# hkust-vgd/scanobjectnn

Measured on AMD Instinct MI355X. Metric: point-clouds/sec fwd+bwd at B×2048×3, 15-cls, higher is better.
Workload: dtype f32

## Files before the change

include/pcops.h:

```cpp
#ifndef PCOPS_H
#define PCOPS_H

#ifdef __cplusplus
extern "C" {
#endif

typedef void *pcops_stream_t;

typedef struct pcops_rows {
    const void *blocks;
    const int *block_start;
    const int *rows;
} pcops_rows_t;

typedef enum pcops_status {
    PCOPS_OK = 0,
    PCOPS_ERR_NULL_POINTER = -1,
    PCOPS_ERR_BAD_SHAPE = -2,
    PCOPS_ERR_BAD_ARGUMENT = -3,
    PCOPS_ERR_UNSUPPORTED = -4,
    PCOPS_ERR_LAUNCH = -5
} pcops_status;

const char *pcops_strerror(int status);
int pcops_abi_version(void);

typedef enum pcops_option {
    PCOPS_OPT_GEMM_SPLIT_BF16 = 1,
    PCOPS_OPT_WGRAD_SPLIT_BF16 = 2,
    PCOPS_OPT_BWD_FUSED_DX_SPLIT_BF16 = 3,
    PCOPS_OPT_KNN_F16_PREFILTER = 4,
    PCOPS_OPT_DGRAD_SPLIT_BF16 = 5,
    PCOPS_OPT_BWD_FUSED_GRAM_WGRAD = 6,
    PCOPS_OPT_SCATTER_QFORM = 7,
    PCOPS_OPT_XYZ_STATS_MOMENTS = 8,
    PCOPS_OPT_GRAM_SPLIT_BF16 = 9,
    PCOPS_OPT_POOL_TOP_ROWS_PIPELINED = 10,
    PCOPS_OPT_XCONV_CHANNEL_GROUPS = 11,
    PCOPS_OPT_COUNT = 12
} pcops_option;
int pcops_set_option(int option, int value);
int pcops_get_option(int option);
int pcops_last_launch_pipe(void);
int pcops_last_launch_plan(int *out, int n);
int pcops_last_launch_acc_stats(void);

int pcops_farthest_point_sample(int b, int n, int m, const float *inp, float *temp,
                                int *out, pcops_stream_t stream);
unsigned long long pcops_farthest_point_sample_workspace_bytes(int b, int n);

int pcops_prob_sample(int b, int n, int m, const float *inp_p, const float *inp_r, float *temp,
                      int *out, pcops_stream_t stream);

int pcops_gather_point(int b, int n, int m, const float *inp, const int *idx,
                       float *out, pcops_stream_t stream);
int pcops_gather_point_grad(int b, int n, int m, const float *out_g, const int *idx,
                            float *inp_g, pcops_stream_t stream);

int pcops_query_ball_point(int b, int n, int m, float radius, int nsample,
                           const float *xyz1, const float *xyz2, int *idx,
                           int *pts_cnt, pcops_stream_t stream);

int pcops_query_ball_point_multi(int b, int n, int m, int nscale, const float *radius,
                                 const int *nsample, const float *xyz1,
                                 const float *xyz2, int *const *idx,
                                 int *const *pts_cnt, pcops_stream_t stream);

int pcops_group_point(int b, int n, int c, int m, int nsample, const float *points,
                      const int *idx, float *out, pcops_stream_t stream);
int pcops_group_point_grad(int b, int n, int c, int m, int nsample,
                           const float *grad_out, const int *idx, float *grad_points,
                           pcops_stream_t stream);

int pcops_selection_sort(int b, int n, int m, int k, const float *dist, int *outi,
                         float *out, pcops_stream_t stream);
int pcops_knn_point_supported(int n);
int pcops_knn_point(int b, int n, int c, int m, int k, const float *xyz1, const float *xyz2, float *val, int *idx,
                    pcops_stream_t stream);
int pcops_knn_point_dist(int b, int n, int c, int m, const float *xyz1, const float *xyz2, float *dist,
                         pcops_stream_t stream);

int pcops_three_nn(int b, int n, int m, const float *xyz1, const float *xyz2,
                   float *dist, int *idx, pcops_stream_t stream);
int pcops_three_interpolate(int b, int m, int c, int n, const float *points,
                            const int *idx, const float *weight, float *out,
                            pcops_stream_t stream);
int pcops_three_interpolate_grad(int b, int n, int c, int m, const float *grad_out,
                                 const int *idx, const float *weight,
                                 float *grad_points, pcops_stream_t stream);

void pcops_set_deterministic(int on);
int pcops_get_deterministic(void);
// ... 415 lines not shown
```

scanobjectnn_amd/_lib.py:

```python
import ctypes as C
import os
import re
import weakref

import torch

_HERE = os.path.dirname(os.path.abspath(__file__))
LIB_PATH = os.environ.get("PCOPS_LIB") or os.path.join(_HERE, "libpcops.so")

_I, _F, _P, _U64, _LL = C.c_int, C.c_float, C.c_void_p, C.c_ulonglong, C.c_longlong
ABI_VERSION = 4

HEADER_PATH = os.path.join(os.path.dirname(_HERE), "include", "pcops.h")


class PcopsError(RuntimeError):
    pass


_SCALARS = {"int": _I, "float": _F, "long long": _LL, "unsigned long long": _U64}


def _ctype(decl, fn):
    if "*" in decl:
# ... 101 lines not shown
def load():
    global _lib
    if _lib is not None:
        return _lib
    if not os.path.exists(LIB_PATH):
        raise PcopsError(
            "libpcops.so is missing (%s). Build it with `python -c 'import __graft_entry__ as g; "
            "g.build()'` or `make -C scanobjectnn_amd/csrc`. There is no CPU fallback." % LIB_PATH)
    lib = C.CDLL(LIB_PATH)
    for name, (argtypes, _) in SIGNATURES.items():
        fn = getattr(lib, name)
        fn.argtypes = list(argtypes) + [_P]
        fn.restype = _I
    for name, (argtypes, restype) in PLAIN.items():
        fn = getattr(lib, name)
        fn.argtypes = argtypes
        fn.restype = restype
    got = int(lib.pcops_abi_version())
    if got != ABI_VERSION:
        raise PcopsError("%s reports ABI version %d, this binding is written for %d: rebuild it "
                         "(make -C scanobjectnn_amd/csrc)" % (LIB_PATH, got, ABI_VERSION))
    _lib = lib
    return lib


def strerror(status):
    return load().pcops_strerror(int(status)).decode()


def ptr(t):
    return t.data_ptr() if t is not None else None


def check(t, dtype, name, ndim=None):
    if not isinstance(t, torch.Tensor):
        raise TypeError("%s must be a torch.Tensor" % name)
    if not t.is_cuda:
        raise PcopsError("%s is on %s: pcops ops run on the MI355X only (no CPU fallback)"
                         % (name, t.device))
    if t.dtype != dtype:
        raise TypeError("%s must be %s, got %s" % (name, dtype, t.dtype))
    if ndim is not None and t.dim() != ndim:
        raise ValueError("%s must have rank %d, got shape %s" % (name, ndim, tuple(t.shape)))
    return t.contiguous()


OPT_GEMM_SPLIT_BF16, OPT_WGRAD_SPLIT_BF16, OPT_BWD_FUSED_DX_SPLIT_BF16, OPT_KNN_F16_PREFILTER = 1, 2, 3, 4
OPT_DGRAD_SPLIT_BF16, OPT_BWD_FUSED_GRAM_WGRAD = 5, 6
OPT_SCATTER_QFORM = 7
OPT_XYZ_STATS_MOMENTS = 8
OPT_GRAM_SPLIT_BF16 = 9
OPT_POOL_TOP_ROWS_PIPELINED = 10
OPT_XCONV_CHANNEL_GROUPS = 11


def set_option(option, value):
    prev = int(load().pcops_set_option(int(option), int(value)))
    if prev < 0:
        raise PcopsError("pcops_set_option(%d, %d): %s" % (option, value, strerror(prev)))
    return prev


def get_option(option):
    return int(load().pcops_get_option(int(option)))


def set_deterministic(on=True):
    load().pcops_set_deterministic(1 if on else 0)


def deterministic():
    return bool(load().pcops_get_deterministic())


def scatter_rows_sorted_supported(rows, ndst):
    return bool(load().pcops_scatter_rows_sorted_supported(int(rows), int(ndst)))


def scatter_rows_sorted(idx, src, ndst, div=1, w=None, out=None, c=None, ld=None, src_ptr=None):
    b, rows = idx.shape[0], idx[0].numel()
    if not scatter_rows_sorted_supported(rows, ndst):
        raise PcopsError("ordered scatter-add (deterministic backward): %d destination points per cloud, the limit is "
                         "%d (the per-cloud counting sort lives in LDS); rows %d must stay below 2^30.  Switch "
                         "deterministic mode off for clouds this large." % (ndst, load().pcops_scatter_rows_sorted_max_ndst(), rows))
    if c is None:
        c, ld = src.shape[-1], src.shape[-1]
    acc = out is not None
    if out is None:
        out = torch.empty((b, ndst, c), dtype=torch.float32, device=idx.device)
    ws = torch.empty(int(load().pcops_scatter_rows_workspace_bytes(b, rows, ndst)) // 8 + 1, dtype=torch.int64,
                     device=idx.device)
    call("pcops_scatter_rows_sorted", b, rows, ndst, c, div, ld, idx.data_ptr(), ptr(w),
         src_ptr if src_ptr is not None else src.data_ptr(), out.data_ptr(), 1 if acc else 0, ws.data_ptr())
    return out


def scatter_grouped(dfg, idx, n):
    b, m, k, c = dfg.shape
    if deterministic():
        return scatter_rows_sorted(idx.view(b, m * k), dfg.view(b, m * k, c), n)
    out = torch.empty((b, n, c), dtype=torch.float32, device=dfg.device)
    call("pcops_group_point_grad", b, n, c, m, k, dfg.data_ptr(), idx.data_ptr(), out.data_ptr())
    return out


_SYNC_EVERY_CALL = os.environ.get("PCOPS_SYNC", "0") == "1"
# ... 19 lines not shown
```

scanobjectnn_amd/csrc/abi.hip:

```cpp
#include <atomic>
#include <cstdint>
#include <cstdlib>

#include "common.h"

extern "C" const char *pcops_strerror(int status) {
    switch (status) {
        case PCOPS_OK: return "ok";
        case PCOPS_ERR_NULL_POINTER: return "null pointer argument";
        case PCOPS_ERR_BAD_SHAPE: return "invalid tensor extents";
        case PCOPS_ERR_BAD_ARGUMENT: return "invalid attribute (radius/nsample/npoint/k)";
        case PCOPS_ERR_UNSUPPORTED: return "shape outside the range the gfx950 kernels are built for";
        case PCOPS_ERR_LAUNCH: return "HIP launch failed";
        default: return "unknown pcops status";
    }
}

extern "C" int pcops_abi_version(void) { return 4; }

static std::atomic<int> g_deterministic{pcops_env_switch("PCOPS_DETERMINISTIC", false) ? 1 : 0};
extern "C" void pcops_set_deterministic(int on) { g_deterministic.store(on ? 1 : 0); }

namespace {
int env_opt(const char *name, int dflt, int hi) {
    const int v = pcops_env_int(name, dflt);
    return v < 0 ? 0 : (v > hi ? hi : v);
}
std::atomic<int> g_options[PCOPS_OPT_COUNT] = {};
std::atomic<int> g_options_init{0};
void options_init() {
    if (g_options_init.load(std::memory_order_acquire)) return;
    static std::atomic_flag busy = ATOMIC_FLAG_INIT;
    while (busy.test_and_set(std::memory_order_acquire)) {}
    if (!g_options_init.load(std::memory_order_relaxed)) {
        g_options[PCOPS_OPT_GEMM_SPLIT_BF16].store(env_opt("PCOPS_GEMM_BF3", 1, 2));
        g_options[PCOPS_OPT_WGRAD_SPLIT_BF16].store(pcops_env_int("PCOPS_WGRAD_BF3", 1) != 0);
        g_options[PCOPS_OPT_BWD_FUSED_DX_SPLIT_BF16].store(env_opt("PCOPS_BWD_FUSED_DX3", 2, 2));
        g_options[PCOPS_OPT_KNN_F16_PREFILTER].store(pcops_env_int("PCOPS_KNN_F16", 1) != 0);
        g_options[PCOPS_OPT_DGRAD_SPLIT_BF16].store(env_opt("PCOPS_DGRAD_BF3", 1, 2));
        g_options[PCOPS_OPT_BWD_FUSED_GRAM_WGRAD].store(pcops_env_int("PCOPS_BWD_FUSED_GW", 0) != 0);
        g_options[PCOPS_OPT_SCATTER_QFORM].store(pcops_env_int("PCOPS_SCATTER_QFORM", 1) != 0);
        g_options[PCOPS_OPT_XYZ_STATS_MOMENTS].store(pcops_env_int("PCOPS_XYZ_STATS_MOMENTS", 0) != 0);
        g_options[PCOPS_OPT_GRAM_SPLIT_BF16].store(pcops_env_int("PCOPS_GRAM_BF3", 1) != 0);
        g_options[PCOPS_OPT_POOL_TOP_ROWS_PIPELINED].store(pcops_env_int("PCOPS_POOL_TOP_ROWS_PIPE", 1) != 0);
        g_options[PCOPS_OPT_XCONV_CHANNEL_GROUPS].store(pcops_env_int("PCOPS_XCONV_GROUPS", 1) != 0);
        g_options_init.store(1, std::memory_order_release);
    }
    busy.clear(std::memory_order_release);
}
}

extern "C" int pcops_get_option(int option) {
    if (option <= 0 || option >= PCOPS_OPT_COUNT) return PCOPS_ERR_BAD_ARGUMENT;
    options_init();
    return g_options[option].load();
}

extern "C" int pcops_set_option(int option, int value) {
    if (option <= 0 || option >= PCOPS_OPT_COUNT || value < 0) return PCOPS_ERR_BAD_ARGUMENT;
    if ((option == PCOPS_OPT_GEMM_SPLIT_BF16 || option == PCOPS_OPT_DGRAD_SPLIT_BF16 ||
         option == PCOPS_OPT_BWD_FUSED_DX_SPLIT_BF16) ? value > 2 : value > 1)
        return PCOPS_ERR_BAD_ARGUMENT;
    options_init();
    return g_options[option].exchange(value);
}
extern "C" int pcops_get_deterministic(void) { return g_deterministic.load(); }

static thread_local int t_last_pipe = 0;
static thread_local int t_last_acc_stats = 0;
void pcops_note_pipe(int pipe) { t_last_pipe = pipe; t_last_acc_stats = 0; }
void pcops_note_acc_stats(int on) { t_last_acc_stats = on; }
extern "C" int pcops_last_launch_pipe(void) { return t_last_pipe; }
extern "C" int pcops_last_launch_acc_stats(void) { return t_last_acc_stats; }

static thread_local int t_last_plan[5] = {0, 0, 0, 0, 0};
void pcops_note_plan(int path, int split, int bn, int wst, int pool) {
    t_last_plan[0] = path; t_last_plan[1] = split; t_last_plan[2] = bn; t_last_plan[3] = wst; t_last_plan[4] = pool;
    t_last_acc_stats = 0;
}
void pcops_note_plan_field(int field, int value) {
    if (field >= 0 && field < 5) t_last_plan[field] = value;
}
extern "C" int pcops_last_launch_plan(int *out, int n) {
    if (!out || n < 0) return PCOPS_ERR_NULL_POINTER;
    for (int i = 0; i < n && i < 5; ++i) out[i] = t_last_plan[i];
    return 5;
}

namespace {
__global__ __launch_bounds__(256) void adam_step_kernel(long long n4, float4 *__restrict__ p, const float4 *__restrict__ g,
                                                        float4 *__restrict__ m, float4 *__restrict__ v, float b1, float b2,
                                                        float lr_t, float eps) {
    const float c1 = 1.f - b1, c2 = 1.f - b2;
    for (long long i = (long long)blockIdx.x * 256 + threadIdx.x; i < n4; i += (long long)gridDim.x * 256) {
        const float4 gi = g[i];
        float4 mi = m[i], vi = v[i], pi = p[i];
        mi.x = fmaf(c1, gi.x, b1 * mi.x); mi.y = fmaf(c1, gi.y, b1 * mi.y);
        mi.z = fmaf(c1, gi.z, b1 * mi.z); mi.w = fmaf(c1, gi.w, b1 * mi.w);
        vi.x = fmaf(c2 * gi.x, gi.x, b2 * vi.x); vi.y = fmaf(c2 * gi.y, gi.y, b2 * vi.y);
        vi.z = fmaf(c2 * gi.z, gi.z, b2 * vi.z); vi.w = fmaf(c2 * gi.w, gi.w, b2 * vi.w);
        pi.x -= lr_t * mi.x / (sqrtf(vi.x) + eps); pi.y -= lr_t * mi.y / (sqrtf(vi.y) + eps);
        pi.z -= lr_t * mi.z / (sqrtf(vi.z) + eps); pi.w -= lr_t * mi.w / (sqrtf(vi.w) + eps);
        m[i] = mi; v[i] = vi; p[i] = pi;
    }
}
__global__ __launch_bounds__(256) void adam_step_dev_kernel(long long n4, float4 *__restrict__ p, const float4 *__restrict__ g,
                                                            float4 *__restrict__ m, float4 *__restrict__ v, float b1, float b2,
                                                            const float *__restrict__ lr_t_dev, float eps) {
    const float c1 = 1.f - b1, c2 = 1.f - b2;
    const float lr_t = *lr_t_dev;
    for (long long i = (long long)blockIdx.x * 256 + threadIdx.x; i < n4; i += (long long)gridDim.x * 256) {
        const float4 gi = g[i];
        float4 mi = m[i], vi = v[i], pi = p[i];
        mi.x = fmaf(c1, gi.x, b1 * mi.x); mi.y = fmaf(c1, gi.y, b1 * mi.y);
// ... 45 lines not shown
```

scanobjectnn_amd/csrc/common.h:

```cpp
#pragma once
#include <hip/hip_runtime.h>
#include <stdint.h>
#include <stdio.h>
#include <stdlib.h>

#include <type_traits>

#include "../../include/pcops.h"
#include "device.h"

#define PCOPS_REQUIRE_PTR(p) \
    do { if ((p) == nullptr) return PCOPS_ERR_NULL_POINTER; } while (0)
#define PCOPS_REQUIRE_SHAPE(cond) \
    do { if (!(cond)) return PCOPS_ERR_BAD_SHAPE; } while (0)
#define PCOPS_REQUIRE_ARG(cond) \
    do { if (!(cond)) return PCOPS_ERR_BAD_ARGUMENT; } while (0)

static inline bool pcops_env_switch(const char *name, bool dflt) {
    const char *e = getenv(name);
    return dflt ? !(e && e[0] == '0') : (e && e[0] == '1');
}
static inline int pcops_env_int(const char *name, int dflt) {
    const char *e = getenv(name);
    return e ? atoi(e) : dflt;
// ... 5 lines not shown
    static const bool verbose = getenv("PCOPS_DEBUG_LAUNCH") != nullptr;
    if (verbose) fprintf(stderr, "libpcops: launch failed: %s (%s)\n", hipGetErrorString(e), hipGetErrorName(e));
    return PCOPS_ERR_LAUNCH;
}

static inline hipStream_t as_stream(pcops_stream_t s) { return reinterpret_cast<hipStream_t>(s); }

static inline unsigned cdiv(long long a, long long b) { return (unsigned)((a + b - 1) / b); }

static __global__ __launch_bounds__(256) void pcops_zero_kernel(unsigned *__restrict__ p, size_t n) {
    for (size_t i = (size_t)blockIdx.x * 256 + threadIdx.x; i < n; i += (size_t)gridDim.x * 256) p[i] = 0u;
}
static inline hipError_t pcops_zero_async(void *p, size_t bytes, hipStream_t st) {
    hipStreamCaptureStatus capturing = hipStreamCaptureStatusNone;
    if (st == nullptr || bytes == 0 || (bytes & 3) || (reinterpret_cast<uintptr_t>(p) & 3) ||
        hipStreamIsCapturing(st, &capturing) != hipSuccess || capturing != hipStreamCaptureStatusActive)
        return hipMemsetAsync(p, 0, bytes, st);
    const size_t n = bytes / 4;
    const unsigned grid = n < (size_t)4096 * 256 ? cdiv((long long)n, 256) : 4096u;
    hipLaunchKernelGGL(pcops_zero_kernel, dim3(grid), dim3(256), 0, st, static_cast<unsigned *>(p), n);
    return hipGetLastError();
}

template <typename... Params, typename... Args>
static inline int pcops_launch_lds(void (*kern)(Params...), dim3 grid, dim3 block, size_t lds, int max_lds, hipStream_t st,
                                   Args... args) {
    if (hipFuncSetAttribute(reinterpret_cast<const void *>(kern), hipFuncAttributeMaxDynamicSharedMemorySize, max_lds) !=
        hipSuccess)
        return PCOPS_ERR_LAUNCH;
    hipLaunchKernelGGL(kern, grid, block, lds, st, args...);
    return pcops_launch_status();
}

template <int... Vs, typename F>
static inline int pcops_dispatch(int v, int otherwise, F &&f) {
    int rc = otherwise;
    (void)((v == Vs && ((rc = f(std::integral_constant<int, Vs>{})), true)) || ...);
    return rc;
}

extern "C" int pcops_get_deterministic(void);
extern "C" int pcops_get_option(int option);
void pcops_note_pipe(int pipe);
void pcops_note_acc_stats(int on);
void pcops_note_plan(int path, int split, int bn, int wst, int pool);
void pcops_note_plan_field(int field, int value);

bool pcops_xyz_bwd_tiles_form(long long M, int K, int N);
int pcops_xyz_bwd_tiles_launch(long long M, int groups, const float *off4, const float *xyzw, const float *a_scale,
                               const float *a_shift, const float *G, const float *Y, const float *p, const float *q,
                               const float *t, const float *W, float *partial, float *dW, float *db, float *stats_partial,
                               float *xyz_stats, hipStream_t st);

constexpr int kWave = 64;

#ifndef PCOPS_WAVE_PRIO
#define PCOPS_WAVE_PRIO 0
#endif
__device__ __forceinline__ void wave_prio_stagger() {
#if PCOPS_WAVE_PRIO & 1
    const unsigned slot = __builtin_amdgcn_s_getreg((3 << 11) | (0 << 6) | 4);
    if (slot & 1) __builtin_amdgcn_s_setprio(1);
#endif
}
__device__ __forceinline__ void wave_prio_consumer(bool consumer) {
#if PCOPS_WAVE_PRIO & 2
    if (consumer) __builtin_amdgcn_s_setprio(1);
#else
    (void)consumer;
#endif
}

__device__ __forceinline__ unsigned wave_max_u32(unsigned v) {
    auto step = [&](auto ctrl, auto rmask) {
        const unsigned o = (unsigned)__builtin_amdgcn_update_dpp(0, (int)v, decltype(ctrl)::value, decltype(rmask)::value,
                                                                 0xf, true);
        v = o > v ? o : v;
    };
    step(std::integral_constant<int, 0x111>{}, std::integral_constant<int, 0xf>{});
    step(std::integral_constant<int, 0x112>{}, std::integral_constant<int, 0xf>{});
    step(std::integral_constant<int, 0x114>{}, std::integral_constant<int, 0xf>{});
    step(std::integral_constant<int, 0x118>{}, std::integral_constant<int, 0xf>{});
    step(std::integral_constant<int, 0x142>{}, std::integral_constant<int, 0xa>{});
    step(std::integral_constant<int, 0x143>{}, std::integral_constant<int, 0xc>{});
    return (unsigned)__builtin_amdgcn_readlane((int)v, 63);
}

__device__ __forceinline__ unsigned long long wave_max_u64(unsigned long long v) {
    const unsigned hi = (unsigned)(v >> 32), lo = (unsigned)(v & 0xffffffffu);
    const unsigned mh = wave_max_u32(hi);
    const unsigned ml = wave_max_u32(hi == mh ? lo : 0u);
    return ((unsigned long long)mh << 32) | ml;
}

__device__ __forceinline__ unsigned xcd_contiguous(unsigned bid, unsigned nwg) {
    const unsigned q = nwg >> 3, r = nwg & 7u, x = bid & 7u, i = bid >> 3;
    return (x < r ? x * (q + 1) : r * (q + 1) + (x - r) * q) + i;
}
struct CloudPart { int part, cloud; };
__device__ __forceinline__ CloudPart xcd_cloud_part() {
    const unsigned vb = xcd_contiguous(blockIdx.x + blockIdx.y * gridDim.x, gridDim.x * gridDim.y);
    const unsigned cloud = vb / gridDim.x;
    return CloudPart{(int)(vb - cloud * gridDim.x), (int)cloud};
}
```

scanobjectnn_amd/csrc/mlp.hip:

```cpp
#include <stdlib.h>

#include "common.h"
#include <initializer_list>
#include <type_traits>

#ifndef PCOPS_MLP_PART
#define PCOPS_MLP_PART (-1)
#endif
#define PCOPS_PART(p_) (PCOPS_MLP_PART < 0 || PCOPS_MLP_PART == (p_))
#define PCOPS_HIDDEN __attribute__((visibility("hidden")))

#ifndef PCOPS_BF_RM
#define PCOPS_BF_RM 1
#endif

namespace pcops_mlp {

constexpr int kBM = 128;
constexpr int kBK = 32;
constexpr int kLdA = 36;

enum AMode { A_PLAIN = 0, A_BNRELU = 1, A_DY = 2, A_DYPOOL = 3, A_DYPOOLU = 4 };
constexpr int A_DYPOOLB = 6;
constexpr int A_DYW = 7;
// ... 5593 lines not shown
    GemmArgs a = fwd_args(M, K, N, nullptr, K, pro_scale, pro_shift, W, bias, Y, stats_partial, stat_pivot);
    a.off4 = off4; a.xw = xyzw; a.xw_ld = K;
    if (const int rc = set_rows(a, rows)) return rc;
    return launch_gemm_ws_only<A_XYZ, E_FWD>(a, as_stream(stream));
}

int pcops_mlp_gemm_dgrad_xyz(int M, int K, int Nout, const float *G, const float *Y, const float *p,
                             const float *q, const float *t, const float *gpool, const unsigned char *argmax,
                             int S, const float *pool_scale, const float *pool_shift, const float *Wt,
                             const float *off4, const float *xyzw, const float *prev_scale,
                             const float *prev_shift, float *Gprev, float *stats_partial, float *xyz_stats,
                             pcops_stream_t stream) {
    return pcops_mlp_gemm_dgrad_xyz_rows(M, K, Nout, G, Y, p, q, t, gpool, argmax, S, pool_scale, pool_shift, Wt, off4,
                                         xyzw, prev_scale, prev_shift, Gprev, stats_partial, xyz_stats, nullptr, stream);
}

int pcops_mlp_gemm_dgrad_xyz_rows(int M, int K, int Nout, const float *G, const float *Y, const float *p,
                                  const float *q, const float *t, const float *gpool, const unsigned char *argmax,
                                  int S, const float *pool_scale, const float *pool_shift, const float *Wt,
                                  const float *off4, const float *xyzw, const float *prev_scale,
                                  const float *prev_shift, float *Gprev, float *stats_partial, float *xyz_stats,
                                  const pcops_rows_t *rows, pcops_stream_t stream) {
    PCOPS_REQUIRE_SHAPE(M >= 1 && K >= 4 && K % 4 == 0 && Nout >= 1);
    PCOPS_REQUIRE_PTR(Y); PCOPS_REQUIRE_PTR(p); PCOPS_REQUIRE_PTR(q); PCOPS_REQUIRE_PTR(t);
    PCOPS_REQUIRE_PTR(Wt); PCOPS_REQUIRE_PTR(off4); PCOPS_REQUIRE_PTR(xyzw);
    PCOPS_REQUIRE_ARG(Gprev != nullptr || xyz_stats != nullptr);
    if (xyz_stats) PCOPS_REQUIRE_PTR(stats_partial);
    PCOPS_REQUIRE_PTR(prev_scale); PCOPS_REQUIRE_PTR(prev_shift);
    if (reinterpret_cast<uintptr_t>(off4) & 15) return PCOPS_ERR_UNSUPPORTED;
    GemmArgs a = {};
    a.M = M; a.K = K; a.N = Nout; a.X = G; a.X2 = Y; a.ldx = K; a.v0 = p; a.v1 = q; a.v2 = t;
    a.v3 = pool_scale; a.v4 = pool_shift; a.gpool = gpool; a.argmax = argmax; a.S = S > 0 ? S : 1;
    a.W = Wt; a.Y = Gprev; a.ldy = Nout; a.msc = prev_scale; a.msh = prev_shift;
    a.off4 = off4; a.xw = xyzw; a.xw_ld = Nout;
    a.stats = stats_partial; a.xstats = xyz_stats;
    if (const int rc = set_rows(a, rows)) return rc;
    hipStream_t st = as_stream(stream);
    if (gpool) {
        PCOPS_REQUIRE_PTR(argmax); PCOPS_REQUIRE_PTR(pool_scale); PCOPS_REQUIRE_PTR(pool_shift);
        a.X = Y;
        return launch_gemm_ws_only<A_DYPOOL, E_MASKX>(a, st);
    }
    PCOPS_REQUIRE_PTR(G);
    return launch_gemm_ws_only<A_DY, E_MASKX>(a, st);
}


static int gram_full_groups(long long M, int K, int ldx, const void *X) {
    if (!gram_full_on() || !ws_enabled() || M < 65536 || K > 320 || K < 32 || K % 4 != 0 || ldx % 4 != 0) return 0;
    if (reinterpret_cast<uintptr_t>(X) & 15) return 0;
    return clamp_groups(256, (M + 31) / 32);
}

int pcops_mlp_wgrad_splits(long long M, int K, int N) {
    WgradPlan pl;
    int best = wgrad_legacy_splits(M, K, N);
    for (const int g : {wgrad_pc_tile(K, N, false, &pl), wgrad_pc_tile(K, N, true, &pl), wgrad_bf3_tile(K, N, &pl),
                        wgrad_ws_tile(K, N, &pl)})
        if (g > best) best = g;
    if (K == N && gram_full_groups(M, K, 4, nullptr) > best) best = gram_full_groups(M, K, 4, nullptr);
    return best;
}

int pcops_gather_stack_rows_supported(int b, int n, int m, int s, int has_q, int nlayers, const int *widths) {
    if (b < 1 || m < 1 || s < kBlk || s % kBlk != 0 || s > 256 || nlayers < 2 || !widths) return 0;
    if (!ws_enabled() || !wgrad_pc_enabled()) return 0;
    const long long M = (long long)b * m * s;
    if (M > 0x7fffffffll) return 0;
    for (int l = 1; l < nlayers; ++l) {
        const int K = widths[l - 1], N = widths[l];
        GemmArgs f = {};
        f.M = (int)M; f.K = K; f.N = N; f.ldx = K; f.ldy = N;
        GemmArgs d = {};
        d.M = (int)M; d.K = N; d.N = K; d.ldx = N; d.ldy = K; d.S = s;
        WsPlan pl;
        if (!ws_plan(f, A_BNRELU, &pl) || !ws_plan(d, A_DY, &pl) || !wgrad_pc_shape_ok(M, K, N, K)) return 0;
    }
    if (has_q && !pcops_sa_scatter_rows_supported(n, m, s, widths[0])) return 0;
    return 1;
}

static int bwd_fused_groups(long long M, int K, int N, int S, int pooled) {
    if (!ws_enabled() || !wgrad_pc_enabled()) return 0;
    static const bool on = pcops_env_switch("PCOPS_BWD_FUSED", true);
    if (!on) return 0;
    if (M < 65536 || M > 0x7fffff00ll || K > 64 || K % 4 != 0 || N > 128 || N % 4 != 0) return 0;
    if (pooled && (S < 1 || S > 255)) return 0;
    return clamp_groups(256, (M + 31) / 32);
}

int pcops_mlp_bwd_fused_groups(long long M, int K, int N, int S, int pooled) { return bwd_fused_groups(M, K, N, S, pooled); }

int pcops_mlp_bwd_fused(long long M, int K, int N, const float *Yprev, const float *a_scale, const float *a_shift,
                        const float *G, const float *Y, const float *p, const float *q, const float *t,
                        const float *gpool, const unsigned char *argmax, int S, const float *W, float *partial,
                        float *dW, float *db, float *Gprev, float *stats_partial, pcops_stream_t stream) {
    return pcops_mlp_bwd_fused_rows(M, K, N, Yprev, a_scale, a_shift, G, Y, p, q, t, gpool, argmax, S, W, partial, dW, db,
                                    Gprev, stats_partial, nullptr, stream);
}


static int bwd_fused_gw_groups(long long M, int K, int N, int S) {
    if (pcops_get_option(PCOPS_OPT_BWD_FUSED_GRAM_WGRAD) == 0 || S < 11 || S > 255) return 0;
    if (pcops_get_option(PCOPS_OPT_BWD_FUSED_DX_SPLIT_BF16) == 0) return 0;
    return bwd_fused_groups(M, K, N, S, 1);
}
// ... 184 lines not shown
    if (!dgrad_top_plan(M, Kp, &pl)) return 0;
    if (!(wgrad_pc_enabled() && wgrad_pc_shape_ok(M, Kp, Kp, Kp, true))) return 0;
    const long long slots = (long long)(M / S) * (S < N ? S : N);
    return slots * Kp * 4 < (long long)kOOB ? 1 : 0;
}

int pcops_mlp_pool_top_addend(int M, int Kp, int N, int S, const float *gout, const float *ysel,
                            const unsigned char *argmax, const float *pool_scale, const float *pool_shift,
                            const float *p, const float *Wt, float *addend, int *rowmap, pcops_stream_t stream) {
    PCOPS_REQUIRE_SHAPE(M >= 1 && S >= 1 && S <= 256 && M % S == 0 && Kp % 4 == 0 && N >= 1 && N <= 65535);
    PCOPS_REQUIRE_PTR(gout); PCOPS_REQUIRE_PTR(ysel); PCOPS_REQUIRE_PTR(argmax); PCOPS_REQUIRE_PTR(pool_scale);
    PCOPS_REQUIRE_PTR(pool_shift); PCOPS_REQUIRE_PTR(p); PCOPS_REQUIRE_PTR(Wt); PCOPS_REQUIRE_PTR(addend);
    PCOPS_REQUIRE_PTR(rowmap);
    if (reinterpret_cast<uintptr_t>(Wt) & 15 || reinterpret_cast<uintptr_t>(addend) & 15) return PCOPS_ERR_UNSUPPORTED;
    if (N > 1024 || Kp > 512) return PCOPS_ERR_UNSUPPORTED;
    if (M / S <= 512)
        hipLaunchKernelGGL(pool_top_addend_kernel<1024>, dim3(M / S), dim3(1024), 0, as_stream(stream), S, N, Kp,
                           S < N ? S : N, gout, ysel, argmax, pool_scale, pool_shift, p, Wt, addend, rowmap);
    else
        hipLaunchKernelGGL(pool_top_addend_kernel<256>, dim3(M / S), dim3(256), 0, as_stream(stream), S, N, Kp,
                           S < N ? S : N, gout, ysel, argmax, pool_scale, pool_shift, p, Wt, addend, rowmap);
    return pcops_launch_status();
}

int pcops_mlp_gemm_dgrad_top(int M, int Kp, const float *Yprev, const float *prev_scale, const float *prev_shift,
                             const float *Mq, const float *vconst, const float *addend, long long addend_rows,
                             const int *rowmap, float *Gprev, float *stats_partial, pcops_stream_t stream) {
    return pcops_mlp_gemm_dgrad_top_rows(M, Kp, Yprev, prev_scale, prev_shift, Mq, vconst, addend, addend_rows, rowmap, Gprev,
                                         stats_partial, nullptr, stream);
}

static int gram_finish(const GramArgs &g, int gg, float *gram, float *xsum, hipStream_t st) {
    const long long L = (long long)g.K * g.K;
    hipLaunchKernelGGL(sum_partials2_kernel, dim3(cdiv(L, 64) + (xsum ? cdiv(g.K, 64) : 0)), dim3(1024), 0, st, gg, L,
                       g.part, gram, (long long)g.K, g.xpart, xsum);
    hipLaunchKernelGGL(mirror_lower_kernel, dim3(g.K), dim3(256), 0, st, g.K, gram);
    return pcops_launch_status();
}

int pcops_mlp_gram(long long M, int Kp, const float *Yprev, int ldx, const float *a_scale, const float *a_shift,
                   float *partial, float *gram, float *xsum, pcops_stream_t stream) {
    PCOPS_REQUIRE_SHAPE(M >= 1 && Kp >= 1 && ldx >= Kp);
    PCOPS_REQUIRE_PTR(Yprev); PCOPS_REQUIRE_PTR(partial); PCOPS_REQUIRE_PTR(gram);
    PCOPS_REQUIRE_ARG((a_scale == nullptr) == (a_shift == nullptr));
    const int gg = gram_full_groups(M, Kp, ldx, Yprev);
    pcops_note_pipe(0);
    if (gg > 0) {
        hipStream_t st = as_stream(stream);
        GramArgs g = {M, Kp, ldx, Yprev, a_scale, a_shift, partial, partial + (long long)gg * Kp * Kp};
        const int nbk = (Kp + 31) / 32;
        const size_t lds = (size_t)(2 * 32 * nbk + 2 * 32 * (32 * nbk + 4)) * sizeof(float);
        const int rc = gram_full_launch(g, nbk, a_scale != nullptr, gg, lds, st);
        return rc ? rc : gram_finish(g, gg, gram, xsum, st);
    }
    WgradArgs a = {};
    a.M = M; a.K = Kp; a.N = Kp;
    a.amode = a_scale ? A_BNRELU : A_PLAIN; a.X = Yprev; a.ldx = ldx; a.asc = a_scale; a.ash = a_shift;
    a.dmode = A_SELFD; a.G = Yprev; a.Y = Yprev; a.ldy = ldx; a.p = a_scale; a.q = a_scale; a.t = a_shift; a.S = 1;
    return wgrad_impl(a, partial, gram, xsum, as_stream(stream));
}

int pcops_mlp_pool_top_wsparse(int M, int Kp, int N, int S, const float *gout, const float *ysel,
                               const unsigned char *argmax, const float *pool_scale, const float *pool_shift,
                               const float *p, const float *Yprev, const float *prev_scale, const float *prev_shift,
                               float *Ssp, float *cfsum, pcops_stream_t stream) {
    PCOPS_REQUIRE_SHAPE(M >= 1 && S >= 1 && S <= 256 && M % S == 0 && Kp >= 1 && Kp <= 512 && N >= 1);
    PCOPS_REQUIRE_PTR(gout); PCOPS_REQUIRE_PTR(ysel); PCOPS_REQUIRE_PTR(argmax); PCOPS_REQUIRE_PTR(pool_scale);
    PCOPS_REQUIRE_PTR(pool_shift); PCOPS_REQUIRE_PTR(p); PCOPS_REQUIRE_PTR(Yprev);
    PCOPS_REQUIRE_ARG((prev_scale == nullptr) == (prev_shift == nullptr));
    PCOPS_REQUIRE_PTR(Ssp); PCOPS_REQUIRE_PTR(cfsum);
    hipLaunchKernelGGL(pool_top_wsparse_kernel, dim3(N), dim3(256), 0, as_stream(stream), (long long)(M / S), S, N,
                       Kp, gout, ysel, argmax, pool_scale, pool_shift, p, Yprev, prev_scale, prev_shift, Ssp, cfsum);
    return pcops_launch_status();
}


static const int kTopRowsWs = 512;

static bool addend_rows_shape_ok(int M, int Kp, int N, int S) {
    return S % kBlk == 0 && S <= 128 && (Kp == 64 || Kp == 128) && N <= 256 && N % 32 == 0 &&
           (long long)M * Kp * 4 < (long long)kOOB;
}

int pcops_mlp_pool_top_rows_supported(int M, int Kp, int N, int S) {
    if (!pcops_mlp_pool_top_supported(M, Kp, N, S)) return 0;
    if (M < 65536 || !addend_rows_shape_ok(M, Kp, N, S)) return 0;
    return gram_full_groups(M, Kp, Kp, nullptr) ? 1 : 0;
}

unsigned long long pcops_mlp_pool_top_wsparse_rows_partial(int Kp, int N) {
    return (unsigned long long)kTopRowsWs * ((unsigned long long)Kp * N + N);
}

int pcops_mlp_pool_top_addend_rows(int M, int Kp, int N, int S, const float *gout, const float *ysel,
                                   const unsigned char *argmax, const float *pool_scale, const float *pool_shift,
                                   const float *p, const float *Wt, float *addend, int *rowmap, const pcops_rows_t *rows,
                                   pcops_stream_t stream) {
    if (!rows) return pcops_mlp_pool_top_addend(M, Kp, N, S, gout, ysel, argmax, pool_scale, pool_shift, p, Wt, addend, rowmap, stream);
    PCOPS_REQUIRE_SHAPE(M >= 1 && S >= 1 && M % S == 0);
    PCOPS_REQUIRE_PTR(gout); PCOPS_REQUIRE_PTR(ysel); PCOPS_REQUIRE_PTR(argmax); PCOPS_REQUIRE_PTR(pool_scale);
    PCOPS_REQUIRE_PTR(pool_shift); PCOPS_REQUIRE_PTR(p); PCOPS_REQUIRE_PTR(Wt); PCOPS_REQUIRE_PTR(addend);
    PCOPS_REQUIRE_PTR(rowmap);
    { const int rrc = rows_ok(rows); if (rrc) return rrc; }
    if (!addend_rows_shape_ok(M, Kp, N, S)) return PCOPS_ERR_UNSUPPORTED;
    if (reinterpret_cast<uintptr_t>(Wt) & 15 || reinterpret_cast<uintptr_t>(addend) & 15) return PCOPS_ERR_UNSUPPORTED;
    const int G = M / S;
// ... 196 lines not shown
```

Measured before the change: 29570.

## Add wide-K gram kernel with split-bf16 MFMA and producer/consumer pipelining

Adds a new gram (X^T X) kernel for channel widths 129–512. It tiles the output into 128x128 block pairs and exploits symmetry by computing only the upper-triangular pairs. Producer waves load fp32 rows, apply the optional BN+ReLU, split each value into three bf16 parts in double-buffered LDS, and compute column sums. Consumer waves accumulate 32x32x16 bf16 MFMA products with separate high and low-order accumulators, which is meant to replace the slower generic wgrad path for wide gram matrices. The path is enabled by default above an M threshold, and adds another kernel with split-precision accuracy trade-offs and large LDS use.

```diff
diff --git a/include/pcops.h b/include/pcops.h
--- a/include/pcops.h
+++ b/include/pcops.h
@@ -37,7 +37,8 @@
     PCOPS_OPT_GRAM_SPLIT_BF16 = 9,
     PCOPS_OPT_POOL_TOP_ROWS_PIPELINED = 10,
     PCOPS_OPT_XCONV_CHANNEL_GROUPS = 11,
-    PCOPS_OPT_COUNT = 12
+    PCOPS_OPT_GRAM_WIDE_SPLIT_BF16 = 12,
+    PCOPS_OPT_COUNT = 13
 } pcops_option;
 int pcops_set_option(int option, int value);
 int pcops_get_option(int option);
diff --git a/scanobjectnn_amd/_lib.py b/scanobjectnn_amd/_lib.py
--- a/scanobjectnn_amd/_lib.py
+++ b/scanobjectnn_amd/_lib.py
@@ -177,6 +177,7 @@
 OPT_GRAM_SPLIT_BF16 = 9
 OPT_POOL_TOP_ROWS_PIPELINED = 10
 OPT_XCONV_CHANNEL_GROUPS = 11
+OPT_GRAM_WIDE_SPLIT_BF16 = 12
 
 
 def set_option(option, value):
diff --git a/scanobjectnn_amd/csrc/abi.hip b/scanobjectnn_amd/csrc/abi.hip
--- a/scanobjectnn_amd/csrc/abi.hip
+++ b/scanobjectnn_amd/csrc/abi.hip
@@ -44,6 +44,7 @@
         g_options[PCOPS_OPT_GRAM_SPLIT_BF16].store(pcops_env_int("PCOPS_GRAM_BF3", 1) != 0);
         g_options[PCOPS_OPT_POOL_TOP_ROWS_PIPELINED].store(pcops_env_int("PCOPS_POOL_TOP_ROWS_PIPE", 1) != 0);
         g_options[PCOPS_OPT_XCONV_CHANNEL_GROUPS].store(pcops_env_int("PCOPS_XCONV_GROUPS", 1) != 0);
+        g_options[PCOPS_OPT_GRAM_WIDE_SPLIT_BF16].store(env_opt("PCOPS_GRAM_WIDE_BF3", 1, 2));
         g_options_init.store(1, std::memory_order_release);
     }
     busy.clear(std::memory_order_release);
@@ -59,7 +60,7 @@
 extern "C" int pcops_set_option(int option, int value) {
     if (option <= 0 || option >= PCOPS_OPT_COUNT || value < 0) return PCOPS_ERR_BAD_ARGUMENT;
     if ((option == PCOPS_OPT_GEMM_SPLIT_BF16 || option == PCOPS_OPT_DGRAD_SPLIT_BF16 ||
-         option == PCOPS_OPT_BWD_FUSED_DX_SPLIT_BF16) ? value > 2 : value > 1)
+         option == PCOPS_OPT_BWD_FUSED_DX_SPLIT_BF16 || option == PCOPS_OPT_GRAM_WIDE_SPLIT_BF16) ? value > 2 : value > 1)
         return PCOPS_ERR_BAD_ARGUMENT;
     options_init();
     return g_options[option].exchange(value);
diff --git a/scanobjectnn_amd/csrc/common.h b/scanobjectnn_amd/csrc/common.h
--- a/scanobjectnn_amd/csrc/common.h
+++ b/scanobjectnn_amd/csrc/common.h
@@ -81,6 +81,10 @@
                                const float *t, const float *W, float *partial, float *dW, float *db, float *stats_partial,
                                float *xyz_stats, hipStream_t st);
 
+int pcops_gram_wide_groups(long long M, int Kp, int max_copies);
+int pcops_gram_wide_launch(long long M, int Kp, const float *X, int ldx, const float *a_scale, const float *a_shift, int groups,
+                           float *part, float *xpart, hipStream_t st);
+
 constexpr int kWave = 64;
 
 #ifndef PCOPS_WAVE_PRIO
diff --git a/scanobjectnn_amd/csrc/gram_wide.hip b/scanobjectnn_amd/csrc/gram_wide.hip
--- /dev/null
+++ b/scanobjectnn_amd/csrc/gram_wide.hip
@@ -0,0 +1,247 @@
+#include "common.h"
+
+namespace {
+
+struct GramWideArgs {
+    long long M;
+    int K, ldx;
+    int G, nblk;
+    const float *X, *asc, *ash;
+    float *part;
+    float *xpart;
+};
+
+constexpr int gw_nb(bool diag, int w) { return diag ? (w < 2 ? 3 : 2) : 4; }
+constexpr int gw_i(bool diag, int w, int b) {
+    return diag ? (w == 0 ? 0 : (w == 1 ? 1 : (w == 2 ? (b == 0 ? 0 : 3) : 2))) : 2 * (w >> 1) + (b >> 1);
+}
+constexpr int gw_j(bool diag, int w, int b) {
+    return diag ? (w == 0 ? b : (w == 1 ? 1 + b : (w == 2 ? 3 : 2 + b))) : 2 * (w & 1) + (b & 1);
+}
+constexpr bool gw_used(bool diag, int w, int side, int blk) {
+    for (int b = 0; b < gw_nb(diag, w); ++b) {
+        if ((diag || side == 0) && gw_i(diag, w, b) == blk) return true;
+        if ((diag || side == 1) && gw_j(diag, w, b) == blk) return true;
+    }
+    return false;
+}
+
+constexpr int kGwRS = 32, kGwRSP = 40, kGwPSZ = 128 * kGwRSP, kGwImg = 3 * kGwPSZ;
+constexpr size_t kGwLds = (size_t)4 * 128 * sizeof(float) + (size_t)2 * 2 * kGwImg * 2;
+
+template <bool DIAG, bool BN>
+__device__ __forceinline__ void gram_wide_pair(const GramWideArgs &a, const int bI, const int bJ, const int grp, float *lds) {
+    constexpr int RS = kGwRS, RSP = kGwRSP, PSZ = kGwPSZ, IMG = kGwImg;
+    constexpr int NIMG = DIAG ? 1 : 2, NV = 4, TBUF = NIMG * IMG;
+    const int tid = threadIdx.x, lane = tid & 63;
+    const int wave = __builtin_amdgcn_readfirstlane(tid >> 6);
+    wave_prio_consumer(wave < 4);
+    const long long M = a.M;
+    const int K = a.K, ngrp = a.G;
+    float *coef = lds;
+    __bf16 *Tp = reinterpret_cast<__bf16 *>(coef + 4 * 128);
+    for (int e = tid; e < 256; e += 512) {
+        const int col = 128 * (e < 128 ? bI : bJ) + (e & 127);
+        const bool in = BN && col < K;
+        coef[(e >> 7) * 256 + (e & 127)] = in ? a.asc[col] : 0.f;
+        coef[(e >> 7) * 256 + 128 + (e & 127)] = in ? a.ash[col] : 0.f;
+    }
+    __syncthreads();
+    const long long nstripes = (M + RS - 1) / RS;
+    const long long cnt = grp < nstripes ? (nstripes - grp + ngrp - 1) / ngrp : 0;
+
+    if (wave >= 4) {
+        const int pt = tid - 256;
+        const int c = (pt & 31) * 4, r0 = pt >> 5;
+        float4 sc[NIMG], sh[NIMG];
+        unsigned voff[NIMG];
+#pragma unroll
+        for (int m = 0; m < NIMG; ++m) {
+            sc[m] = *reinterpret_cast<const float4 *>(&coef[m * 256 + c]);
+            sh[m] = *reinterpret_cast<const float4 *>(&coef[m * 256 + 128 + c]);
+            const int col = 128 * (m == 0 ? bI : bJ) + c;
+            voff[m] = col < K ? (unsigned)(r0 * a.ldx + col) * 4u : kOOB;
+        }
+        const unsigned rstep = (unsigned)(8 * a.ldx) * 4u;
+        float4 pxa[NIMG * NV], pxb[NIMG * NV];
+        float cs[NV][4];
+#pragma unroll
+        for (int j = 0; j < NV; ++j) cs[j][0] = cs[j][1] = cs[j][2] = cs[j][3] = 0.f;
+        auto issue = [&](float4 (&px)[NIMG * NV], long long stripe) {
+            const long long row0 = stripe * RS;
+            const long long left = M - row0 < RS ? M - row0 : RS;
+            const __amdgpu_buffer_rsrc_t rx = make_rsrc(a.X + row0 * a.ldx, left * a.ldx * 4);
+#pragma unroll
+            for (int m = 0; m < NIMG; ++m)
+#pragma unroll
+                for (int j = 0; j < NV; ++j) px[m * NV + j] = buf_load4(rx, voff[m] + (unsigned)j * rstep, 0u);
+        };
+        auto stage = [&](const float4 (&px)[NIMG * NV], long long stripe, __bf16 *dst) {
+            const long long row0 = stripe * RS;
+#pragma unroll
+            for (int m = 0; m < NIMG; ++m) {
+                float4 xt[NV];
+#pragma unroll
+                for (int j = 0; j < NV; ++j) {
+                    float4 x = px[m * NV + j];
+                    if (BN) {
+                        x.x = fmaxf(fmaf(x.x, sc[m].x, sh[m].x), 0.f); x.y = fmaxf(fmaf(x.y, sc[m].y, sh[m].y), 0.f);
+                        x.z = fmaxf(fmaf(x.z, sc[m].z, sh[m].z), 0.f); x.w = fmaxf(fmaf(x.w, sc[m].w, sh[m].w), 0.f);
+                        if (!(row0 + r0 + 8 * j < M)) x = make_float4(0.f, 0.f, 0.f, 0.f);
+                    }
+                    if (DIAG) { cs[j][0] += x.x; cs[j][1] += x.y; cs[j][2] += x.z; cs[j][3] += x.w; }
+                    xt[j] = x;
+                }
+#pragma unroll
+                for (int e = 0; e < 4; ++e) {
+                    const float v0 = e == 0 ? xt[0].x : (e == 1 ? xt[0].y : (e == 2 ? xt[0].z : xt[0].w));
+                    const float v1 = e == 0 ? xt[1].x : (e == 1 ? xt[1].y : (e == 2 ? xt[1].z : xt[1].w));
+                    const float v2 = e == 0 ? xt[2].x : (e == 1 ? xt[2].y : (e == 2 ? xt[2].z : xt[2].w));
+                    const float v3 = e == 0 ? xt[3].x : (e == 1 ? xt[3].y : (e == 2 ? xt[3].z : xt[3].w));
+                    bf16x2 h0, m0, l0, h1, m1, l1;
+                    split3_pair(v0, v1, h0, m0, l0);
+                    split3_pair(v2, v3, h1, m1, l1);
+                    __bf16 *d = dst + m * IMG + (32 * e + (c >> 2)) * RSP + 4 * r0;
+                    const bf16x4 hv = {h0.x, h0.y, h1.x, h1.y}, mv = {m0.x, m0.y, m1.x, m1.y}, lv = {l0.x, l0.y, l1.x, l1.y};
+                    *reinterpret_cast<bf16x4 *>(d) = hv;
+                    *reinterpret_cast<bf16x4 *>(d + PSZ) = mv;
+                    *reinterpret_cast<bf16x4 *>(d + 2 * PSZ) = lv;
+                }
+            }
+        };
+        issue(pxa, grp);
+        issue(pxb, grp + ngrp);
+        if (cnt > 0) stage(pxa, grp, Tp);
+        issue(pxa, grp + 2ll * ngrp);
+        __syncthreads();
+        long long i = 0;
+        for (; i + 2 < cnt; i += 2) {
+            stage(pxb, grp + (i + 1) * ngrp, Tp + TBUF);
+            __builtin_amdgcn_sched_barrier(0);
+            issue(pxb, grp + (i + 3) * ngrp);
+            __syncthreads();
+            __builtin_amdgcn_sched_barrier(0);
+            stage(pxa, grp + (i + 2) * ngrp, Tp);
+            __builtin_amdgcn_sched_barrier(0);
+            issue(pxa, grp + (i + 4) * ngrp);
+            __syncthreads();
+            __builtin_amdgcn_sched_barrier(0);
+        }
+        if (i + 1 < cnt) {
+            stage(pxb, grp + (i + 1) * ngrp, Tp + TBUF);
+            __syncthreads();
+        }
+        if (cnt > 0) __syncthreads();
+        if (DIAG) {
+            float *scr = reinterpret_cast<float *>(Tp);
+#pragma unroll
+            for (int j = 0; j < NV; ++j)
+                *reinterpret_cast<float4 *>(&scr[(pt + 256 * j) * 4]) = make_float4(cs[j][0], cs[j][1], cs[j][2], cs[j][3]);
+            __syncthreads();
+            if (pt < 128 && 128 * bI + pt < K) {
+                float sum = 0.f;
+                for (int idx = pt >> 2; idx < 256 * NV; idx += 32) sum += scr[idx * 4 + (pt & 3)];
+                a.xpart[(long long)grp * K + 128 * bI + pt] = sum;
+            }
+            __syncthreads();
+        }
+    } else {
+        const int half = lane >> 5, li = lane & 31;
+        auto run = [&](auto wv_) {
+            constexpr int WV = decltype(wv_)::value;
+            constexpr int NB_ = gw_nb(DIAG, WV);
+            f32x16 acc[NB_], sm[NB_];
+#pragma unroll
+            for (int b = 0; b < NB_; ++b)
+#pragma unroll
+                for (int v = 0; v < 16; ++v) acc[b][v] = sm[b][v] = 0.f;
+            __syncthreads();
+            for (long long i = 0; i < cnt; ++i) {
+                const __bf16 *tb = Tp + (i & 1) * TBUF + li * RSP + 8 * half;
+#pragma unroll
+                for (int s = 0; s < 2; ++s) {
+                    bf16x8 f[2][4][3];
+#pragma unroll
+                    for (int side = 0; side < NIMG; ++side)
+#pragma unroll
+                        for (int blk = 0; blk < 4; ++blk)
+#pragma unroll
+                            for (int pc = 0; pc < 3; ++pc)
+                                if (gw_used(DIAG, WV, side, blk))
+                                    f[side][blk][pc] =
+                                        *reinterpret_cast<const bf16x8 *>(tb + side * IMG + pc * PSZ + 32 * blk * RSP + 16 * s);
+                    __builtin_amdgcn_sched_barrier(0);
+#define PCOPS_GWMM(A_, B_, C_)                                                                                       \
+    _Pragma("unroll") for (int b = 0; b < NB_; ++b)                                                                  \
+        C_[b] = __builtin_amdgcn_mfma_f32_32x32x16_bf16(f[0][gw_i(DIAG, WV, b)][A_], f[DIAG ? 0 : 1][gw_j(DIAG, WV, b)][B_], \
+                                                        C_[b], 0, 0, 0)
+                    PCOPS_GWMM(2, 0, sm);
+                    PCOPS_GWMM(0, 2, sm);
+                    PCOPS_GWMM(1, 1, sm);
+                    PCOPS_GWMM(1, 0, sm);
+                    PCOPS_GWMM(0, 1, sm);
+                    PCOPS_GWMM(0, 0, acc);
+#undef PCOPS_GWMM
+                    __builtin_amdgcn_sched_barrier(0);
+                }
+                __syncthreads();
+            }
+            float *out = a.part + (long long)grp * K * K;
+#pragma unroll
+            for (int b = 0; b < NB_; ++b) {
+                const int si = gw_i(DIAG, WV, b), sj = gw_j(DIAG, WV, b);
+                const int cb = 128 * bJ + 4 * li + sj;
+#pragma unroll
+                for (int v = 0; v < 16; ++v) {
+                    const int ca = 128 * bI + 4 * ((v & 3) + 8 * (v >> 2) + 4 * half) + si;
+                    const float val = acc[b][v] + sm[b][v];
+                    if (ca < K && cb < K) {
+                        out[(long long)ca * K + cb] = val;
+                        if (!DIAG || si != sj) out[(long long)cb * K + ca] = val;
+                    }
+                }
+            }
+            if (DIAG) {
+                __syncthreads();
+                __syncthreads();
+            }
+        };
+        if (wave == 0) run(std::integral_constant<int, 0>{});
+        else if (wave == 1) run(std::integral_constant<int, 1>{});
+        else if (wave == 2) run(std::integral_constant<int, 2>{});
+        else run(std::integral_constant<int, 3>{});
+    }
+}
+
+template <bool BN>
+__global__ __launch_bounds__(512, 1) void gram_wide_bf3_kernel(GramWideArgs a) {
+    extern __shared__ __attribute__((aligned(16))) float lds[];
+    const int npairs = a.nblk * (a.nblk + 1) / 2;
+    const int vb = (int)xcd_contiguous(blockIdx.x, gridDim.x);
+    const int grp = __builtin_amdgcn_readfirstlane(vb / npairs);
+    int u = __builtin_amdgcn_readfirstlane(vb - grp * npairs), bI = 0;
+    while (u >= a.nblk - bI) { u -= a.nblk - bI; ++bI; }
+    const int bJ = bI + u;
+    if (bI == bJ) gram_wide_pair<true, BN>(a, bI, bJ, grp, lds);
+    else gram_wide_pair<false, BN>(a, bI, bJ, grp, lds);
+}
+
+}
+
+int pcops_gram_wide_groups(long long M, int Kp, int max_copies) {
+    const int nblk = (Kp + 127) / 128;
+    long long g = 256 / (nblk * (nblk + 1) / 2);
+    const long long nstripes = (M + kGwRS - 1) / kGwRS;
+    if (g > nstripes) g = nstripes;
+    if (g > max_copies) g = max_copies;
+    return g < 1 ? 1 : (int)g;
+}
+
+int pcops_gram_wide_launch(long long M, int Kp, const float *X, int ldx, const float *a_scale, const float *a_shift, int groups,
+                           float *part, float *xpart, hipStream_t st) {
+    const int nblk = (Kp + 127) / 128;
+    GramWideArgs a = {M, Kp, ldx, groups, nblk, X, a_scale, a_shift, part, xpart};
+    const dim3 grid(groups * nblk * (nblk + 1) / 2);
+    return a_scale ? pcops_launch_lds(gram_wide_bf3_kernel<true>, grid, dim3(512), kGwLds, 160 * 1024, st, a)
+                   : pcops_launch_lds(gram_wide_bf3_kernel<false>, grid, dim3(512), kGwLds, 160 * 1024, st, a);
+}
diff --git a/scanobjectnn_amd/csrc/mlp.hip b/scanobjectnn_amd/csrc/mlp.hip
--- a/scanobjectnn_amd/csrc/mlp.hip
+++ b/scanobjectnn_amd/csrc/mlp.hip
@@ -5669,6 +5669,14 @@
     return clamp_groups(256, (M + 31) / 32);
 }
 
+static int gram_wide_groups(long long M, int K, int ldx, const void *X) {
+    const int opt = pcops_get_option(PCOPS_OPT_GRAM_WIDE_SPLIT_BF16);
+    if (opt == 0 || (opt != 2 && M < (K <= 256 ? 32768 : 16384)) || gram_full_groups(M, K, ldx, X) > 0) return 0;
+    if (K <= 128 || K > 512 || K % 64 != 0 || ldx % 4 != 0 || (reinterpret_cast<uintptr_t>(X) & 15)) return 0;
+    WgradPlan pl;
+    return pcops_gram_wide_groups(M, K, wgrad_pc_tile(K, K, false, &pl));
+}
+
 int pcops_mlp_wgrad_splits(long long M, int K, int N) {
     WgradPlan pl;
     int best = wgrad_legacy_splits(M, K, N);
@@ -5959,6 +5967,15 @@
         const size_t lds = (size_t)(2 * 32 * nbk + 2 * 32 * (32 * nbk + 4)) * sizeof(float);
         const int rc = gram_full_launch(g, nbk, a_scale != nullptr, gg, lds, st);
         return rc ? rc : gram_finish(g, gg, gram, xsum, st);
+    }
+    if (const int gw = gram_wide_groups(M, Kp, ldx, Yprev)) {
+        hipStream_t st = as_stream(stream);
+        GramArgs g = {M, Kp, ldx, Yprev, a_scale, a_shift, partial, partial + (long long)gw * Kp * Kp};
+        const int rc = pcops_gram_wide_launch(M, Kp, Yprev, ldx, a_scale, a_shift, gw, g.part, g.xpart, st);
+        if (rc) return rc;
+        pcops_note_pipe(1);
+        pcops_note_plan(18, 1, 128, gw, 0);
+        return gram_finish(g, gw, gram, xsum, st);
     }
     WgradArgs a = {};
     a.M = M; a.K = Kp; a.N = Kp;
```

After: 29810, median of 6. About the same (+0.8%).
